# alexkroman/tiny-audio

Measured on AMD Instinct MI355X. Metric: training audio-sec/sec on 10s@16kHz clips, higher is better.
Workload: dtype bf16

## Files before the change

### include/ta355.h

```cpp
#ifndef TA355_H
#define TA355_H

#ifdef __cplusplus
extern "C" {
#endif

#ifndef __HIP_PLATFORM_AMD__
typedef struct ihipStream_t* hipStream_t;
#endif

#define TA_OK 0
#define TA_ERR_ARG 1
#define TA_ERR_LAUNCH 2

int ta_version(void);



long ta_logmel_scratch_floats(int B, int Ls, int n_mels);
int ta_logmel_mel_ranges(const float* melfb, int n_mels, int* mel_ranges, hipStream_t st);
int ta_logmel_f32(const float* wav, const long* lens, int B, int Ls, const float* dft, const float* window,
                  const float* melfb, int n_mels, float* feats, int* mask, float* scratch, const int* mel_ranges, hipStream_t st);

typedef struct {
// ... 224 lines not shown
                             const int* kmask, const int* seg, int B, int Hq, int Hkv, int L, float scale, float eps,
                             hipStream_t st);
int ta_attention_bwd_seg(const void* Q, const void* K, const void* V, const void* dO, long dO_stride, const float* LSE,
                         const float* Delta, const int* kmask, const int* seg, void* dQ, void* dK, void* dV, int B, int Hq,
                         int Hkv, int L, int Lp, float scale, hipStream_t st);
int ta_attention_bwd_qkv_seg(const void* Q, const void* K, const void* V, const void* dO, long dO_stride, const float* LSE,
                             const float* Delta, const int* kmask, const int* seg, const void* qkv0, const float* rq,
                             const float* rk, const float* qn_w, const float* kn_w, const float* cosT, const float* sinT,
                             const int* pos, void* dqkv, int B, int Hq, int Hkv, int L, int Lp, float scale, hipStream_t st);
int ta_lora_dropout_keep(const ta_lora_dropout* drop, int layer, int linear, int M, int in, unsigned char* out, hipStream_t st);


int ta_attention_enc_fwd(const void* qkv, void* out, int B, int heads, int S, hipStream_t st);

int ta_gemm_bf16_nt(const void* A, const void* W, void* C, int M, int N, int K, long lda, int a_rpb, long a_bs,
                    long ldc, int c_rpb, long c_bs, long c_off, const float* bias, const float* residual, int act,
                    int out_bf16, int splits, float* splitk_ws, hipStream_t st);
int ta_gemm_bf16_nt_ex(const void* A, const void* W, void* C, int M, int N, int K, long lda, int a_rpb, long a_bs,
                       long ldc, int c_rpb, long c_bs, long c_off, const float* bias, const float* residual, int act,
                       int out_bf16, int splits, float* splitk_ws, const int* a_idx, const int* seg,
                       const int* krange, hipStream_t st);
typedef struct {
  const void* a2; const void* w2; int k2; long lda2;
  const void* residual_bf16;
  const float* rope_tab; int rope_rows;
  int w_blocked;
  int rope_cols;
} ta_gemm_opts;
int ta_gemm_bf16_nt_opt(const void* A, const void* W, void* C, int M, int N, int K, long lda, int a_rpb, long a_bs,
                        long ldc, int c_rpb, long c_bs, long c_off, const float* bias, const float* residual, int act,
                        int out_bf16, int splits, float* splitk_ws, const int* a_idx, const int* seg,
                        const int* krange, const ta_gemm_opts* opts, hipStream_t st);
long ta_gemm_splitk_ws_bytes(int M, int N, int splits);
int ta_gemm_bf16_nt_grouped(const void* A, const void* W, void* C, int M, int N, int K, const float* bias, int act, int out_bf16,
                            const int* a_idx, const int* seg, const int* krange, int n_groups, long w_stride, long c_stride,
                            hipStream_t st);
long ta_gemm_bf16_tn_ws_bytes(int M, int Ny, int Nx);
int ta_gemm_bf16_tn(const void* Y, const void* X, float* out, int M, int Ny, int Nx, int accumulate, void* ws, long ws_bytes,
                    hipStream_t st);
int ta_profile_gemm(int enable);
int ta_profile_gemm_collect(double* total_ms, double* total_flops, long* launches);
long ta_profile_gemm_log(long* out, long max_rows);
int ta_gemm_reload_knobs(void);

int ta_layernorm_f32(const float* x, const float* w, const float* b, void* y_bf16, float* y_f32,
                     const float* rowscale, int M, int H, float eps, hipStream_t st);
int ta_layernorm_bf16(const void* x_bf16, const float* w, const float* b, void* y_bf16, float* y_f32, const float* rowscale,
                      int M, int H, float eps, hipStream_t st);
int ta_rmsnorm_fwd(const float* x, const float* w, void* y_bf16, float* y_f32, float* rstd, int M, int H,
                   float eps, int act_gelu, hipStream_t st);
int ta_rmsnorm_bwd(const float* dy, const float* x, const float* rstd, const float* w, const float* dres,
                   float* dx_f32, void* dx_bf16, float* dw_accum, int M, int H, int act_gelu, hipStream_t st);
int ta_rmsnorm_fwd_bf16(const void* x_bf16, const float* w, void* y_bf16, float* y_f32, float* rstd, int M, int H, float eps,
                        hipStream_t st);
int ta_rmsnorm_bwd_bf16(const void* dy, int dy_is_bf16, const void* x_bf16, const float* rstd, const float* w,
                        const float* dres, float* dx_f32, void* dx_bf16, int M, int H, hipStream_t st);
int ta_rmsnorm_bwd_bf16s(const void* dy, int dy_is_bf16, const void* x_bf16, const float* rstd, const float* w,
                         const void* dres_bf16, float* dx_f32, void* dx_bf16, int M, int H, hipStream_t st);
int ta_rmsnorm_bwd_dyb(const void* dy_bf16, const float* x, const float* rstd, const float* w, const float* dres, float* dx_f32,
                       void* dx_bf16, int M, int H, hipStream_t st);

int ta_rmsnorm_dw(const void* dy, int dy_is_bf16, const void* x, int x_is_bf16, const float* rstd, float* dw_accum, int M,
                  int H, hipStream_t st);

int ta_attention_fwd(const void* Q, const void* K, const void* VT, void* O, float* LSE, const int* kmask, int B,
                     int Hq, int Hkv, int L, int Lp, int head_dim, int causal, float scale, hipStream_t st);
// ... 81 lines not shown
```

### tiny_audio_amd/csrc/api.hip

```cpp
#include <cstdlib>
#include "common.h"
#include "internal.h"
#include "../../include/ta355.h"

extern "C" int ta_version(void) { return 4; }

#include <algorithm>
#include "host_util.h"


namespace {
struct EncDesc {
  int H, F, L, nh, NM, max_pos, k1;
  float eps;
  const void *conv1_w, *conv2_w;
  const float *conv1_b, *conv2_b, *norm_w, *norm_b;
  const float *rope_cos, *rope_sin, *rope_il, *pos_emb;
  const ta_enc_layer* layers;
  int res_f32;
  bool whisper;
};
EncDesc enc_desc(const ta_encoder_weights* w) {
  return EncDesc{w->hidden, w->ffn, w->n_layers, w->heads, w->n_mels, w->max_pos, 3 * w->n_mels, w->ln_eps, w->conv1_w, w->conv2_w,
                 w->conv1_b, w->conv2_b, w->norm_w, w->norm_b, w->rope_cos, w->rope_sin, w->rope_il, nullptr, w->layers, w->res_f32, false};
// ... 271 lines not shown
  s.xn = c.take<bf16_t>((size_t)d.M * d.D);
  s.act = c.take<bf16_t>((size_t)d.M * d.F);
  s.hl = c.take<bf16_t>((size_t)nl * d.D);
  s.logits = c.take<float>((size_t)nl * w->vocab_pad);
  s.dhl = c.take<float>((size_t)nl * d.D);
  s.dhn = c.take<float>((size_t)d.M * d.D);
  s.dxa = c.take<float>((size_t)d.M * d.D);
  s.dxb32 = c.take<float>((size_t)d.M * d.D);
  s.dxn = c.take<float>((size_t)d.M * d.D);
  s.dxb = c.take<bf16_t>((size_t)d.M * d.D);
  s.dact = c.take<bf16_t>((size_t)d.M * d.F);
  s.dgu = c.take<bf16_t>((size_t)d.M * 2 * d.F);
  s.dao = c.take<bf16_t>((size_t)d.M * d.nq * d.hd);
  s.dot = nullptr;
  s.delta = c.take<float>((size_t)B * d.nq * L);
  s.dq = c.take<bf16_t>((size_t)d.M * d.nq * d.hd);
  s.dk = c.take<bf16_t>((size_t)d.M * d.nkv * d.hd);
  s.dv = c.take<bf16_t>((size_t)d.M * d.nkv * d.hd);
  s.dqkv = c.take<bf16_t>((size_t)d.M * d.NQKV);
  s.dyB = c.take<bf16_t>((size_t)d.M * 64);
  s.lora_part = nullptr; s.lp_layer = 0;
  if (w->lora_rank > 0) {
    const int r = w->lora_rank, bq = d.nq * d.hd;
    const int members[4] = {3, 1, 2, 1}, Ng[4] = {d.NQKV, d.D, 2 * d.F, d.D}, ing[4] = {d.D, bq, d.D, d.F};
    long off = 0;
    for (int g = 0; g < 4; ++g) {
      const int chunks = ta_cdiv((int)d.M, ta_i_lora_tn2_rows((int)d.M, Ng[g], ing[g]));
      s.lp_size[2 * g] = (long)members[g] * r * ing[g]; s.lp_size[2 * g + 1] = (long)Ng[g] * r;
      for (int h = 0; h < 2; ++h) { s.lp_chunks[2 * g + h] = chunks; s.lp_off[2 * g + h] = off; off += s.lp_size[2 * g + h] * chunks; }
    }
    s.lp_layer = off;
    s.lora_part = c.take<float>((size_t)off * w->n_layers);
  }
  const int sp = pick_splits(nl, d.D, w->vocab_pad);
  s.skws = c.take<float>((size_t)ta_gemm_splitk_ws_bytes(nl, d.D, sp) / 4 + 4);
  s.tA = s.tB = nullptr; s.wsk = nullptr;
  if (w->train_base) {
    const int Kp = pad64((int)d.M), Kl = pad64(nl), bq = d.nq * d.hd;
    const size_t a_rows = (size_t)std::max(std::max(2 * d.F, d.NQKV), d.D), b_rows = (size_t)std::max(std::max(d.F, bq), d.D);
    s.tA = c.take<bf16_t>(std::max(a_rows * Kp, (size_t)w->vocab_pad * Kl));
    s.tB = c.take<bf16_t>(std::max(b_rows * Kp, (size_t)d.D * Kl));
    const int shp[4][2] = {{d.NQKV, d.D}, {d.D, bq}, {2 * d.F, d.D}, {d.D, d.F}};
    size_t mx = 0;
    for (auto& q : shp) {
      mx = std::max(mx, (size_t)ta_gemm_splitk_ws_bytes(q[0], q[1], wgrad_splits(q[0], q[1], Kp)));
      mx = std::max(mx, (size_t)ta_gemm_bf16_tn_ws_bytes((int)d.M, q[0], q[1]));
    }
    s.wsk = c.take<float>(mx / 4 + 4);
  }
  s.bytes = c.total();
  return s;
}
}

extern "C" long ta_lm_tape_bytes(const ta_lm_weights* w, int B, int L, int n_label_rows) {
  LmLayerTape store[MAX_LM_LAYERS];
  if (w->n_layers > MAX_LM_LAYERS) return -1;
  return (long)lm_tape(w, B, L, n_label_rows, nullptr, store).bytes;
}
extern "C" long ta_lm_workspace_bytes(const ta_lm_weights* w, int B, int L, int n_label_rows) {
  return (long)lm_ws(w, B, L, n_label_rows, nullptr).bytes;
}

static int lm_layers_forward(const ta_lm_weights* w, const LmDims& d, int B, int L, const int* kmask, const int* pos,
                             LmLayerTape* store, bool alias, float* x_final, LmWs& s, const ta_i_lora_layer_imgs* ext,
                             bf16_t* kcache, bf16_t* vcache, int Lmax, hipStream_t st, const LoraDropDev* drop = nullptr,
                             const int* seg = nullptr) {
// ... 296 lines not shown
  }
  if (n_lab <= 0) {
    if (d_embeds && hipMemsetAsync(d_embeds, 0, (size_t)M * d.D * 4, st) != hipSuccess) return TA_ERR_LAUNCH;
    return TA_OK;
  }
  ta_gemm_opts kx = opts_none();
  LoraDrop pend{};
  const bf16_t* pend_at = nullptr;
  auto lora_bwd = [&](const bf16_t* dy, int N, const bf16_t* x, int in, const bf16_t* xa, const LoraImg& g, float* dla,
                      float* dlb, int members, int b0, int b1, int layer, int grp) -> int {
    static const int lj_base[4] = {0, 3, 4, 6};
    RC(ta_i_lora_skinny_nt(dy, N, g.bt, s.dyB, M, members * r, st));
    float* pb = lora_parts ? s.lora_part + (long)layer * s.lp_layer + s.lp_off[2 * grp + 1] : nullptr;
    float* pa = lora_parts ? s.lora_part + (long)layer * s.lp_layer + s.lp_off[2 * grp] : nullptr;
    if (dp) {
      pend = LoraDrop{*dp, (unsigned)(8 * layer + lj_base[grp]), r, members};
      RC(ta_i_lora_skinny_tn2(dy, N, xa, members * r, dlb, r, 1, 1.0f, r, b0, b1, x, in, s.dyB, members * r, dla, 1, in,
                              w->lora_scale * dp->inv_keep, 0, 0, 0, M, pb, s.lp_size[2 * grp + 1], pa, s.lp_size[2 * grp], st, &pend));
      pend_at = g.at;
      return TA_OK;
    }
    RC(ta_i_lora_skinny_tn2(dy, N, xa, members * r, dlb, r, 1, 1.0f, r, b0, b1, x, in, s.dyB, members * r, dla, 1, in, w->lora_scale,
                            0, 0, 0, M, pb, s.lp_size[2 * grp + 1], pa, s.lp_size[2 * grp], st));
    kx = opts_kext(s.dyB, g.at);
    return TA_OK;
  };
  auto take_ext = [&]() { const ta_gemm_opts o = kx; kx = opts_none(); return o; };
  auto dx_drop_term = [&](void* out, int in) -> int {
    if (!pend_at) return TA_OK;
    const bf16_t* at = pend_at;
    pend_at = nullptr;
    return ta_i_lora_dx_drop(s.dyB, at, out, M, in, pend, st);
  };
  const int sp = pick_splits(n_lab, d.D, w->vocab_pad);
  RC(ta_gemm_bf16_nt(t.dlogits, w->embed_t_bf16, s.dhl, n_lab, d.D, w->vocab_pad, w->vocab_pad, 0, 0, d.D, 0, 0, 0, nullptr,
                     nullptr, 0, 0, sp, s.skws, st));
  if (hipMemsetAsync(s.dhn, 0, (size_t)M * d.D * 4, st) != hipSuccess) return TA_ERR_LAUNCH;
  RC(ta_scatter_rows_f32(s.dhl, label_rows, s.dhn, n_lab, d.D, st));
  const int Kp = pad64(M);
  auto wgrad = [&](const bf16_t* dy, int n_out, const bf16_t* x, int k_in, float* dW) -> int {
    if (!dW) return TA_OK;
    if (n_out <= 4096 && k_in <= 2048)
      return ta_gemm_bf16_tn(dy, x, dW, M, n_out, k_in, 1, s.wsk, ta_gemm_bf16_tn_ws_bytes(M, n_out, k_in), st);
    RC(ta_transpose_to_bf16(dy, 0, n_out, 0, 0, s.tA, Kp, M, n_out, st));
    RC(ta_transpose_to_bf16(x, 0, k_in, 0, 0, s.tB, Kp, M, k_in, st));
    return ta_gemm_bf16_nt(s.tA, s.tB, dW, n_out, k_in, Kp, Kp, 0, 0, k_in, 0, 0, 0, nullptr, dW, 0, 0,
                           wgrad_splits(n_out, k_in, Kp), s.wsk, st);
  };
  if (wg) {
    if (wg->dembed) {
      const int Kl = pad64(n_lab);
      RC(ta_gather_rows_bf16(t.hn, label_rows, s.hl, n_lab, d.D, st));
      RC(ta_transpose_to_bf16(t.dlogits, 0, w->vocab_pad, 0, 0, s.tA, Kl, n_lab, w->vocab_pad, st));
      RC(ta_transpose_to_bf16(s.hl, 0, d.D, 0, 0, s.tB, Kl, n_lab, d.D, st));
      RC(ta_gemm_bf16_nt(s.tA, s.tB, wg->dembed, w->vocab, d.D, Kl, Kl, 0, 0, d.D, 0, 0, 0, nullptr, wg->dembed, 0, 0, 1,
                         nullptr, st));
    }
    if (wg->dnorm) RC(ta_rmsnorm_dw(s.dhn, 0, t.x_final, lm_res_bf16(w), t.r_f, wg->dnorm, M, d.D, st));
  }
  float* dx = s.dxa;
  float* dx_alt = s.dxb32;
  const int gb = 1;
  const bool dx_bf16 = lm_res_bf16(w) && w->dx_f32 == 0;
  auto norm_bwd = [&](const float* dy, int dyb, const float* x, const float* r, const float* gw, const float* dres, float* dxf,
                      bool last = false) -> int {
    if (dx_bf16) return ta_rmsnorm_bwd_bf16s(dy, dyb, x, r, gw, dres ? s.dxb : nullptr, last ? dxf : nullptr, s.dxb, M, d.D, st);
    if (lm_res_bf16(w)) return ta_rmsnorm_bwd_bf16(dy, dyb, x, r, gw, dres, dxf, s.dxb, M, d.D, st);
// ... 68 lines not shown
```

### tiny_audio_amd/csrc/common.h

```cpp
#pragma once
#include <hip/hip_runtime.h>
#include <stdint.h>

typedef uint16_t bf16_t;
typedef __attribute__((ext_vector_type(8))) short bf16x8;
typedef __attribute__((ext_vector_type(4))) short bf16x4;
typedef __attribute__((ext_vector_type(4))) float f32x4;

#define TA_OK 0
#define TA_ERR_ARG 1
#define TA_ERR_LAUNCH 2

#define TA_LAUNCH(...)                \
  do {                                \
    (void)hipGetLastError();          \
    hipLaunchKernelGGL(__VA_ARGS__);  \
  } while (0)

#define TA_CHECK_LAUNCH()                                  \
  do {                                                     \
    hipError_t e__ = hipGetLastError();                    \
    if (e__ != hipSuccess) return TA_ERR_LAUNCH;           \
  } while (0)

__device__ __forceinline__ float bf2f(bf16_t v) { return __uint_as_float(((uint32_t)v) << 16); }

typedef __attribute__((ext_vector_type(2))) __bf16 ta_bf2_t;
typedef __attribute__((ext_vector_type(2))) float ta_f2_t;
__device__ __forceinline__ uint32_t pack2bf(float lo, float hi) {
  ta_f2_t v = {lo, hi};
  ta_bf2_t b = __builtin_convertvector(v, ta_bf2_t);
  return __builtin_bit_cast(uint32_t, b);
}
__device__ __forceinline__ bf16_t f2bf(float f) { return (bf16_t)(pack2bf(f, 0.f) & 0xffffu); }

__device__ __forceinline__ float wave_sum(float v) {
#pragma unroll
  for (int o = 32; o > 0; o >>= 1) v += __shfl_xor(v, o, 64);
  return v;
}
__device__ __forceinline__ float wave_max(float v) {
#pragma unroll
  for (int o = 32; o > 0; o >>= 1) v = fmaxf(v, __shfl_xor(v, o, 64));
  return v;
}

__device__ __forceinline__ float gelu_erf(float x) { return 0.5f * x * (1.0f + erff(x * 0.70710678118654752f)); }
__device__ __forceinline__ float gelu_erf_grad(float x) {
  return 0.5f * (1.0f + erff(x * 0.70710678118654752f)) + x * 0.3989422804014327f * __expf(-0.5f * x * x);
}

__device__ __forceinline__ float gelu_erf_fast(float x) {
  const float z = x * 0.70710678118654752f, az = fabsf(z);
  const float t = __builtin_amdgcn_rcpf(fmaf(0.3275911f, az, 1.0f));
  float p = fmaf(1.061405429f, t, -1.453152027f);
  p = fmaf(p, t, 1.421413741f);
  p = fmaf(p, t, -0.284496736f);
  p = fmaf(p, t, 0.254829592f);
  const float e = __builtin_amdgcn_exp2f(-az * az * 1.4426950408889634f);
  const float erfz = copysignf(1.0f - p * t * e, z);
  return 0.5f * x * (1.0f + erfz);
}

static inline int ta_cdiv(long a, long b) { return (int)((a + b - 1) / b); }
```

### tiny_audio_amd/csrc/elementwise.hip

```cpp
#include "common.h"

static inline int ew_blocks(long n, int per_block = 256) {
  long b = (n + per_block - 1) / per_block;
  return (int)(b > 4096 ? 4096 : (b < 1 ? 1 : b));
}

__global__ void swiglu_fwd_kernel(const bf16_t* __restrict__ gu, bf16_t* __restrict__ act, long M, int F) {
  const long n4 = M * (F / 4);
  for (long i = (long)blockIdx.x * blockDim.x + threadIdx.x; i < n4; i += (long)gridDim.x * blockDim.x) {
    const long m = i / (F / 4); const int c = (int)(i % (F / 4)) * 4;
    const uint2 gv = *(const uint2*)(gu + m * 2 * F + c);
    const uint2 uv = *(const uint2*)(gu + m * 2 * F + F + c);
    const float g[4] = {bf2f(gv.x & 0xffff), bf2f(gv.x >> 16), bf2f(gv.y & 0xffff), bf2f(gv.y >> 16)};
    const float u[4] = {bf2f(uv.x & 0xffff), bf2f(uv.x >> 16), bf2f(uv.y & 0xffff), bf2f(uv.y >> 16)};
    float a[4];
#pragma unroll
    for (int j = 0; j < 4; ++j) a[j] = g[j] / (1.f + __expf(-g[j])) * u[j];
    uint2 o; o.x = pack2bf(a[0], a[1]); o.y = pack2bf(a[2], a[3]);
    *(uint2*)(act + m * F + c) = o;
  }
}
__global__ void swiglu_bwd_kernel(const bf16_t* __restrict__ dact, const bf16_t* __restrict__ gu,
                                  bf16_t* __restrict__ dgu, long M, int F) {
  const long n4 = M * (F / 4);
// ... 112 lines not shown

template <bool F32>
__global__ __launch_bounds__(256) void pos_add_kernel(void* __restrict__ xv, const float* __restrict__ pos, long n_chunks, long per_clip) {
  for (long i = (long)blockIdx.x * blockDim.x + threadIdx.x; i < n_chunks; i += (long)gridDim.x * blockDim.x) {
    const long j = i % per_clip;
    if constexpr (F32) {
      float4 v = ((const float4*)xv)[i];
      const float4 p = ((const float4*)pos)[j];
      v.x += p.x; v.y += p.y; v.z += p.z; v.w += p.w;
      ((float4*)xv)[i] = v;
    } else {
      const uint4 v = ((const uint4*)xv)[i];
      const float4 p0 = ((const float4*)pos)[2 * j], p1 = ((const float4*)pos)[2 * j + 1];
      uint4 o;
      o.x = pack2bf(bf2f(v.x & 0xffff) + p0.x, bf2f(v.x >> 16) + p0.y);
      o.y = pack2bf(bf2f(v.y & 0xffff) + p0.z, bf2f(v.y >> 16) + p0.w);
      o.z = pack2bf(bf2f(v.z & 0xffff) + p1.x, bf2f(v.z >> 16) + p1.y);
      o.w = pack2bf(bf2f(v.w & 0xffff) + p1.z, bf2f(v.w >> 16) + p1.w);
      ((uint4*)xv)[i] = o;
    }
  }
}
extern "C" int ta_pos_add(void* x, int x_f32, const float* pos, int B, int S, int H, hipStream_t st) {
  if (B <= 0 || S <= 0) return TA_OK;
  if (!x || !pos || H <= 0 || (H % 8)) return TA_ERR_ARG;
  const long per_clip = (long)S * H / (x_f32 ? 4 : 8), n = per_clip * B;
  if (x_f32) TA_LAUNCH((pos_add_kernel<true>), dim3(ew_blocks(n)), dim3(256), 0, st, x, pos, n, per_clip);
  else TA_LAUNCH((pos_add_kernel<false>), dim3(ew_blocks(n)), dim3(256), 0, st, x, pos, n, per_clip);
  TA_CHECK_LAUNCH(); return TA_OK;
}

__global__ __launch_bounds__(1024) void audio_index_kernel(const long* __restrict__ ids, const long* __restrict__ counts,
                                                           int* __restrict__ src_row, int B, int L, int N, long audio_id) {
  __shared__ int scan[1024];
  __shared__ int carry;
  __shared__ long cum[1025];
  const int tid = threadIdx.x;
  if (tid == 0) {
    carry = 0; cum[0] = 0;
    for (int i = 0; i < B && i < 1024; ++i) cum[i + 1] = cum[i] + counts[i];
  }
  __syncthreads();
  const int total = B * L;
  for (int base = 0; base < total; base += 1024) {
    const int p = base + tid;
    const int flag = (p < total && ids[p] == audio_id) ? 1 : 0;
    scan[tid] = flag;
    __syncthreads();
    for (int o = 1; o < 1024; o <<= 1) {
      const int v = tid >= o ? scan[tid - o] : 0;
      __syncthreads();
      scan[tid] += v;
      __syncthreads();
    }
    if (p < total) {
      int out = -1;
      if (flag) {
        const long rank = carry + scan[tid] - 1;
        int lo = 0, hi = B;
        while (hi - lo > 1) { const int mid = (lo + hi) >> 1; if (cum[mid] <= rank) lo = mid; else hi = mid; }
        const long n = rank - cum[lo];
        out = (rank < cum[B] && n < N) ? (int)(lo * N + n) : -2;
      }
      src_row[p] = out;
    }
    __syncthreads();
    if (tid == 1023) carry += scan[1023];
    __syncthreads();
  }
}
__global__ __launch_bounds__(256) void segment_table_kernel(const int* __restrict__ sid, int* __restrict__ seg_start,
                                                            int* __restrict__ seg_end, int* __restrict__ pos, int R, int L) {
  const long p = (long)blockIdx.x * 256 + threadIdx.x;
  if (p >= (long)R * L) return;
  const int l = (int)(p % L);
  const int* row = sid + (p - l);
  const int s = row[l];
  int a = l, e = l + 1;
  if (s == 0) { a = l + 1; e = l; }
  else {
    while (a > 0 && row[a - 1] == s) --a;
    while (e < L && row[e] == s) ++e;
  }
  seg_start[p] = a;
  seg_end[p] = e;
  if (pos) pos[p] = s == 0 ? 0 : l - a;
}
__global__ __launch_bounds__(256) void audio_index_seg_kernel(const long* __restrict__ ids, const int* __restrict__ sid,
                                                              const long* __restrict__ counts, int* __restrict__ src_row, int R, int L,
                                                              int C_, int N, long audio_id) {
  __shared__ int clip0;
  const int r = blockIdx.x;
  if (threadIdx.x == 0) {
    int c = 0;
    for (int i = 0; i < r; ++i) { int m = 0; for (int l = 0; l < L; ++l) m = max(m, sid[(long)i * L + l]); c += m; }
    clip0 = c;
  }
  __syncthreads();
  const int* srow = sid + (long)r * L;
  const long* irow = ids + (long)r * L;
  for (int l = threadIdx.x; l < L; l += 256) {
// ... 218 lines not shown
```

### tiny_audio_amd/csrc/gemm.hip

```cpp
#include "gemm_common.h"

template <int ACT, bool OUT_BF16, bool HAS_RES, int BMT = 128, bool KEXT = false>
__global__ __launch_bounds__(256, 2) void gemm_nt_kernel(GemmArgs p) {
  constexpr int MI = BMT / 32, WR = BMT / 2;
  __shared__ __attribute__((aligned(16))) char smem[4 * TILE_BYTES];
  const int tid = threadIdx.x, lane = tid & 63, wave = tid >> 6;
  const int wm = wave >> 1, wn = wave & 1;
  const int g = lane >> 4, l15 = lane & 15;

  const int nwg = gridDim.x;
  int bid = blockIdx.x;
  {
    const int q = nwg >> 3, r = nwg & 7, xcd = bid & 7, within = bid >> 3;
    bid = (xcd < r ? xcd * (q + 1) : r * (q + 1) + (xcd - r) * q) + within;
  }
  const int tiles = p.tiles_m * p.tiles_n;
  const int z = bid / tiles;
  int t = bid - z * tiles;
  const int GROUP_M = p.group_m > 0 ? p.group_m : 8;
  const int width = GROUP_M * p.tiles_n;
  const int group = t / width;
  const int first_m = group * GROUP_M;
  const int gsize = min(p.tiles_m - first_m, GROUP_M);
  int pm = first_m + (t % width) % gsize;
// ... 642 lines not shown
  const bool wide = epilogue_wide_ok(p);
  const float2* lut = stage_gelu_lut<ACT, 256>(smem, p, tid, true);
  if (res_init) epilogue_tile<6, 4, ACT, OUT_BF16, false>(acc, p, Cb, m0 + wm * 96 + l15, Mact, rbase, n0 + wn * 64, g, wide, biasp, lut);
  else epilogue_tile<6, 4, ACT, OUT_BF16, HAS_RES, ((HAS_RES && !OUT_BF16) ? 3 : 2)>(acc, p, Cb, m0 + wm * 96 + l15, Mact, rbase, n0 + wn * 64, g, wide, biasp, lut);
}

#include <vector>
namespace {
struct ProfRec { hipEvent_t a, b; double flops; };
bool g_prof_on = false;
std::vector<ProfRec> g_prof;
#define TA_GEMM_LOG_FIELDS 24
bool g_log_on = false;
std::vector<long> g_log;
}

#include <cstdlib>
struct GemmKnobs {
  int variant;
  int gelu_erf;
  void load() {
    auto i = [](const char* n, int d) { const char* v = getenv(n); return (v && *v) ? atoi(v) : d; };
    variant = i("TA355_GEMM_VARIANT", -1);
    gelu_erf = i("TA355_GELU_LUT", 1) == 0;
  }
};
static GemmKnobs& knobs() {
  static GemmKnobs k = [] { GemmKnobs x; x.load(); return x; }();
  return k;
}
void ta_i_reload_decode_knobs();
extern "C" int ta_gemm_reload_knobs(void) { knobs().load(); ta_i_reload_decode_knobs(); return TA_OK; }

static int pick_variant(int M, int N, int K, int splits) {
  const int forced = knobs().variant;
  if (forced >= 0 && forced <= 12 && !(forced >= 6 && forced <= 9) && forced != 11) return forced;
  const double rate[6] = {1.0, TA355_RATE_256x256, TA355_RATE_256x128, TA355_RATE_256x256_PP, TA355_RATE_256x320_PP, TA355_RATE_96x128};
  const int bm[6] = {128, 256, 256, 256, 256, 96}, bn[6] = {128, 256, 128, 256, 320, 128}, slots[6] = {512, 256, 256, 256, 256, 512};
  int best = 0; double best_t = 1e300;
  for (int v = 0; v < 6; ++v) {
    const long tiles = (long)ta_cdiv(M, bm[v]) * ta_cdiv(N, bn[v]) * splits;
    const double rounds = (double)((tiles + slots[v] - 1) / slots[v]);
    const double t = rounds * (double)bm[v] * bn[v] / rate[v] * ((v == 0 || v == 5) ? 2.0 : 1.0);
    if (t < best_t) { best_t = t; best = v; }
  }
  {
    const long tiles = (long)ta_cdiv(M, 192) * ta_cdiv(N, 128) * splits;
    const double t = (double)((tiles + 255) / 256) * 192.0 * 128.0 / TA355_RATE_192x128;
    if (TA355_RATE_192x128 > 0.0 && K / splits >= 2048 && t < best_t) { best_t = t; best = 10; }
  }
  {
    const long tiles = (long)ta_cdiv(M, 192) * ta_cdiv(N, 256) * splits;
    const double t = (double)((tiles + 255) / 256) * 192.0 * 256.0 / TA355_RATE_192x256_PP;
    if (TA355_RATE_192x256_PP > 0.0 && K / splits >= 128 && t < best_t) { best_t = t; best = 12; }
  }
  return best;
}

template <int ACT, bool OUT_BF16, bool HAS_RES, bool KEXT>
static void launch_variant(int variant, bool persist, int grid, int pgrid, const GemmArgs& a, hipStream_t st) {
  if (variant == 0) TA_LAUNCH((gemm_nt_kernel<ACT, OUT_BF16, HAS_RES, 128, KEXT>), dim3(grid), dim3(256), 0, st, a);
  else if (variant == 5) TA_LAUNCH((gemm_nt_kernel<ACT, OUT_BF16, HAS_RES, 96, KEXT>), dim3(grid), dim3(256), 0, st, a);
  else if (variant == 1) TA_LAUNCH((gemm_nt_kernel_v2<256, ACT, OUT_BF16, HAS_RES, false, KEXT>), dim3(grid), dim3(512), 0, st, a);
  else if (variant == 12) TA_LAUNCH((gemm_nt_kernel_v4<256, ACT, OUT_BF16, HAS_RES, 192>), dim3(pgrid), dim3(512), 0, st, a);
  else if (variant == 3 && persist) TA_LAUNCH((gemm_nt_kernel_v4<256, ACT, OUT_BF16, HAS_RES>), dim3(pgrid), dim3(512), 0, st, a);
  else if (variant == 4 && persist) TA_LAUNCH((gemm_nt_kernel_v4<320, ACT, OUT_BF16, HAS_RES>), dim3(pgrid), dim3(512), 0, st, a);
  else if (variant == 3) TA_LAUNCH((gemm_nt_kernel_v2<256, ACT, OUT_BF16, HAS_RES, true, KEXT>), dim3(grid), dim3(512), 0, st, a);
  else if (variant == 4) TA_LAUNCH((gemm_nt_kernel_v2<320, ACT, OUT_BF16, HAS_RES, true, KEXT>), dim3(grid), dim3(512), 0, st, a);
  else if (variant == 10) TA_LAUNCH((gemm_nt_kernel_v5<ACT, OUT_BF16, HAS_RES, KEXT>), dim3(grid), dim3(256), 0, st, a);
  else TA_LAUNCH((gemm_nt_kernel_v2<128, ACT, OUT_BF16, HAS_RES, false, KEXT>), dim3(grid), dim3(512), 0, st, a);
}

template <int ACT, bool OUT_BF16, bool HAS_RES>
static int launch_gemm(GemmArgs a, hipStream_t st) {
  if (a.A2 && ACT != 0) return TA_ERR_ARG;
  int variant = pick_variant(a.M, a.N, a.K, a.splits);
  const bool a_far = !a.a_plain && ((long)(a.M / a.a_rpb + 1) * a.a_bs + a.lda * a.a_rpb) * 2 >= (1L << 32);
  if (variant == 10 && (a.w_blocked || a.a_idx || a_far)) variant = 5;
  if (variant == 12 && (a.a_idx || a_far || a.A2)) variant = 3;
  const int bm = variant == 0 ? 128 : (variant == 5 ? 96 : ((variant == 10 || variant == 12) ? 192 : 256));
  const int bn = variant == 4 ? 320 : ((variant == 1 || variant == 3 || variant == 12) ? 256 : 128);
  a.tiles_m = ta_cdiv(a.M, bm) + ((a.grp_n > 0 && a.seg) ? a.grp_n : 0); a.tiles_n = ta_cdiv(a.N, bn);
  const int grid = a.tiles_m * a.tiles_n * a.splits;
  a.group_m = (variant != 0 && a.tiles_m <= 8) ? a.tiles_m : 0;
  a.wide = (((long)a.N | a.ldc | a.c_off | a.c_bs) & 7) == 0;
  a.gelu_erf = knobs().gelu_erf;
  const bool persist = (variant == 3 || variant == 4) && !a.a_idx && !a.A2 && !a_far;
  static const int ncu = [] { int dev = 0, n = 0; (void)hipGetDevice(&dev); (void)hipDeviceGetAttribute(&n, hipDeviceAttributeMultiprocessorCount, dev); return n > 0 ? n : 256; }();
  const int pgrid = grid < ncu ? grid : ncu;
// ... 168 lines not shown
```

### tiny_audio_amd/csrc/host_util.h

```cpp
#pragma once
#include "common.h"
#include "internal.h"
#include "../../include/ta355.h"

namespace {
struct Carver {
  char* base; size_t off;
  explicit Carver(void* b) : base((char*)b), off(0) {}
  template <typename T> T* take(size_t n) {
    off = (off + 255) & ~(size_t)255;
    T* p = base ? (T*)(base + off) : nullptr;
    off += n * sizeof(T);
    return p;
  }
  size_t total() const { return (off + 255) & ~(size_t)255; }
};
inline int pad64(int x) { return (x + 63) / 64 * 64; }
inline int gemm(const void* A, const void* W, void* C, int M, int N, int K, const float* bias, const float* res, int act,
                int out_bf16, hipStream_t st) {
  return ta_gemm_bf16_nt(A, W, C, M, N, K, K, 0, 0, N, 0, 0, 0, bias, res, act, out_bf16, 1, nullptr, st);
}
inline int gemm_opt(const void* A, const void* W, void* C, int M, int N, int K, const float* bias, const float* res, int act,
                    int out_bf16, const ta_gemm_opts& o, hipStream_t st) {
  return ta_gemm_bf16_nt_opt(A, W, C, M, N, K, K, 0, 0, N, 0, 0, 0, bias, res, act, out_bf16, 1, nullptr, nullptr, nullptr, nullptr,
                             &o, st);
}
inline ta_gemm_opts opts_none() { return ta_gemm_opts{nullptr, nullptr, 0, 0, nullptr, nullptr, 0, 0, 0}; }
inline ta_gemm_opts opts_kext(const void* a2, const void* w2) { ta_gemm_opts o = opts_none(); o.a2 = a2; o.w2 = w2; o.k2 = 64; o.lda2 = 64; return o; }
inline int pick_splits(int M, int N, int K) {
  const long tiles = (long)ta_cdiv(M, 128) * ta_cdiv(N, 128);
  int s = 1;
  while (tiles * s < 512 && K / 64 / (s * 2) >= 8 && s < 64) s *= 2;
  return s;
}
#define RC(x) do { int rc__ = (x); if (rc__) return rc__; } while (0)
inline size_t lora_imgs_carve(const ta_lm_weights* w, void* base, ta_i_lora_layer_imgs* out) {
  Carver c(base);
  const int D = w->hidden, F = w->ffn, bq = w->heads * w->head_dim, NQKV = (w->heads + 2 * w->kv_heads) * w->head_dim;
  const int in[4] = {D, bq, D, F}, N[4] = {NQKV, D, 2 * F, D};
  for (int l = 0; l < w->n_layers; ++l)
    for (int g = 0; g < 4; ++g) {
      LoraImg im;
      im.a = c.take<bf16_t>((size_t)64 * in[g]); im.at = c.take<bf16_t>((size_t)64 * in[g]);
      im.b = c.take<bf16_t>((size_t)64 * N[g]); im.bt = c.take<bf16_t>((size_t)64 * N[g]);
      if (out) out[l].g[g] = im;
    }
  return c.total();
}
}
```

### tiny_audio_amd/csrc/loss.hip

```cpp
#include "common.h"

template <typename T> __device__ __forceinline__ float4 ld4(const T* p);
template <> __device__ __forceinline__ float4 ld4<float>(const float* p) { return *(const float4*)p; }
template <> __device__ __forceinline__ float4 ld4<bf16_t>(const bf16_t* p) {
  const uint2 v = *(const uint2*)p;
  return make_float4(bf2f(v.x & 0xffff), bf2f(v.x >> 16), bf2f(v.y & 0xffff), bf2f(v.y >> 16));
}

template <typename T>
__global__ __launch_bounds__(256) void ce_fwd_bwd_kernel(const T* __restrict__ logits, long ldl, const int* __restrict__ rows,
                                                         const long* __restrict__ targets, int V, float scale,
                                                         float* __restrict__ nll_out, float* __restrict__ loss_accum,
                                                         bf16_t* __restrict__ dlogits, long ldd) {
  __shared__ float red_m[4], red_s[4];
  const int i = blockIdx.x, tid = threadIdx.x, lane = tid & 63, wave = tid >> 6;
  const long tgt = targets[i];
  const T* row = logits + (long)(rows ? rows[i] : i) * ldl;
  const int nv = V / 4;
  float m = -INFINITY, s = 0.f;
  for (int c = tid; c < nv; c += 256) {
    const float4 v = ld4<T>(row + c * 4);
    const float mx = fmaxf(fmaxf(v.x, v.y), fmaxf(v.z, v.w));
    if (mx > m) { s *= __expf(m - mx); m = mx; }
    s += __expf(v.x - m) + __expf(v.y - m) + __expf(v.z - m) + __expf(v.w - m);
  }
  for (int c = nv * 4 + tid; c < V; c += 256) {
    const float v = sizeof(T) == 4 ? (float)((const float*)row)[c] : bf2f(((const bf16_t*)row)[c]);
    if (v > m) { s *= __expf(m - v); m = v; }
    s += __expf(v - m);
  }
#pragma unroll
  for (int o = 32; o > 0; o >>= 1) {
    const float m2 = __shfl_xor(m, o, 64), s2 = __shfl_xor(s, o, 64);
    const float mn = fmaxf(m, m2);
    s = (m == -INFINITY ? 0.f : s * __expf(m - mn)) + (m2 == -INFINITY ? 0.f : s2 * __expf(m2 - mn));
    m = mn;
  }
  if (lane == 0) { red_m[wave] = m; red_s[wave] = s; }
  __syncthreads();
  float M = fmaxf(fmaxf(red_m[0], red_m[1]), fmaxf(red_m[2], red_m[3]));
  float S = 0.f;
#pragma unroll
  for (int w = 0; w < 4; ++w) S += red_m[w] == -INFINITY ? 0.f : red_s[w] * __expf(red_m[w] - M);
  const float lse = M + __logf(S);
  const bool valid = tgt >= 0 && tgt < V;
  if (tid == 0) {
    float nll = 0.f;
    if (valid) {
      const float zt = sizeof(T) == 4 ? (float)((const float*)row)[tgt] : bf2f(((const bf16_t*)row)[tgt]);
      nll = lse - zt;
      if (loss_accum) atomicAdd(loss_accum, nll * scale);
    }
    if (nll_out) nll_out[i] = nll;
  }
  if (!dlogits) return;
  bf16_t* drow = dlogits + (long)i * ldd;
  const float sc = valid ? scale : 0.f;
  const int nvd = (int)(ldd / 4);
  for (int c = tid; c < nvd; c += 256) {
    float o[4] = {0.f, 0.f, 0.f, 0.f};
    if (c * 4 + 3 < V) {
      const float4 v = ld4<T>(row + c * 4);
      o[0] = __expf(v.x - lse) * sc; o[1] = __expf(v.y - lse) * sc; o[2] = __expf(v.z - lse) * sc; o[3] = __expf(v.w - lse) * sc;
    } else {
      for (int j = 0; j < 4; ++j) {
        const int cc = c * 4 + j;
        if (cc < V) {
          const float v = sizeof(T) == 4 ? (float)((const float*)row)[cc] : bf2f(((const bf16_t*)row)[cc]);
          o[j] = __expf(v - lse) * sc;
        }
      }
    }
    if (valid && (long)c * 4 <= tgt && tgt < (long)c * 4 + 4) o[tgt - (long)c * 4] -= sc;
    uint2 w; w.x = pack2bf(o[0], o[1]); w.y = pack2bf(o[2], o[3]);
    *(uint2*)(drow + c * 4) = w;
  }
}

__global__ __launch_bounds__(1024) void label_rows_kernel(const long* __restrict__ labels, int B, int L,
                                                          int* __restrict__ rows, long* __restrict__ targets,
                                                          int* __restrict__ n_out) {
  __shared__ int scan[1024];
  __shared__ int carry;
  const int tid = threadIdx.x;
  if (tid == 0) carry = 0;
  __syncthreads();
  const int total = B * L;
  for (int base = 0; base < total; base += 1024) {
    const int p = base + tid;
    long t = -100;
    if (p < total) { const int l = p % L; if (l + 1 < L) t = labels[p + 1]; }
    const int flag = (t != -100) ? 1 : 0;
    scan[tid] = flag;
    __syncthreads();
    for (int o = 1; o < 1024; o <<= 1) {
      const int v = tid >= o ? scan[tid - o] : 0;
      __syncthreads();
      scan[tid] += v;
      __syncthreads();
    }
    if (flag) { const int k = carry + scan[tid] - 1; rows[k] = p; targets[k] = t; }
    __syncthreads();
    if (tid == 1023) carry += scan[1023];
    __syncthreads();
  }
  if (tid == 0) n_out[0] = carry;
}

__global__ __launch_bounds__(1024) void nll_sum_kernel(const float* __restrict__ nll, int n, float scale, float* __restrict__ loss_accum) {
  __shared__ float red[16];
  float s = 0.f;
  for (int i = threadIdx.x; i < n; i += 1024) s += nll[i] * scale;
  s = wave_sum(s);
  if ((threadIdx.x & 63) == 0) red[threadIdx.x >> 6] = s;
  __syncthreads();
  if (threadIdx.x == 0) {
    float t = 0.f;
    for (int w = 0; w < 16; ++w) t += red[w];
    loss_accum[0] += t;
  }
}

extern "C" int ta_cross_entropy(const void* logits, int logits_bf16, long ldl, const int* rows, const long* targets,
                                int n, int V, float scale, float* nll, float* loss_accum, void* dlogits_bf16, long ldd,
                                hipStream_t st) {
  if (n <= 0) return TA_OK;
  if ((ldl % 4) || (dlogits_bf16 && (ldd % 4))) return TA_ERR_ARG;
  float* atomic_loss = nll ? nullptr : loss_accum;
  if (logits_bf16)
    TA_LAUNCH((ce_fwd_bwd_kernel<bf16_t>), dim3(n), dim3(256), 0, st, (const bf16_t*)logits, ldl, rows, targets, V,
                       scale, nll, atomic_loss, (bf16_t*)dlogits_bf16, ldd);
  else
    TA_LAUNCH((ce_fwd_bwd_kernel<float>), dim3(n), dim3(256), 0, st, (const float*)logits, ldl, rows, targets, V,
                       scale, nll, atomic_loss, (bf16_t*)dlogits_bf16, ldd);
  TA_CHECK_LAUNCH();
  if (loss_accum && nll) {
    TA_LAUNCH(nll_sum_kernel, dim3(1), dim3(1024), 0, st, nll, n, scale, loss_accum);
    TA_CHECK_LAUNCH();
  }
// ... 10 lines not shown
```

Measured before the change: 7599.

## Add cost-model split-K planner, wave-level block scans, and unrolled CE loops

Adds a split-K planner that scores candidate split counts with the variant cost model plus a reduction penalty, and uses it for the LM-head dgrad GEMM. Replaces the serial 1024-wide shared-memory Hillis-Steele scans in label_rows and audio_index with a two-level wavefront shuffle scan, each thread handling a contiguous chunk. Unrolls the cross-entropy forward and backward loops 8-way so several loads are in flight at once, and simplifies the target check. The scan changes cut sync-heavy small kernels; the split-K change may alter GEMM time and the size of the workspace it needs.

```diff
diff --git a/include/ta355.h b/include/ta355.h
--- a/include/ta355.h
+++ b/include/ta355.h
@@ -280,6 +280,7 @@
                         int out_bf16, int splits, float* splitk_ws, const int* a_idx, const int* seg,
                         const int* krange, const ta_gemm_opts* opts, hipStream_t st);
 long ta_gemm_splitk_ws_bytes(int M, int N, int splits);
+int ta_gemm_plan(int M, int N, int K, int splits_default, int* variant, int* splits);
 int ta_gemm_bf16_nt_grouped(const void* A, const void* W, void* C, int M, int N, int K, const float* bias, int act, int out_bf16,
                             const int* a_idx, const int* seg, const int* krange, int n_groups, long w_stride, long c_stride,
                             hipStream_t st);
diff --git a/tiny_audio_amd/csrc/api.hip b/tiny_audio_amd/csrc/api.hip
--- a/tiny_audio_amd/csrc/api.hip
+++ b/tiny_audio_amd/csrc/api.hip
@@ -327,7 +327,7 @@
     s.lp_layer = off;
     s.lora_part = c.take<float>((size_t)off * w->n_layers);
   }
-  const int sp = pick_splits(nl, d.D, w->vocab_pad);
+  const int sp = pick_splits_plain(nl, d.D, w->vocab_pad);
   s.skws = c.take<float>((size_t)ta_gemm_splitk_ws_bytes(nl, d.D, sp) / 4 + 4);
   s.tA = s.tB = nullptr; s.wsk = nullptr;
   if (w->train_base) {
@@ -690,7 +690,7 @@
     pend_at = nullptr;
     return ta_i_lora_dx_drop(s.dyB, at, out, M, in, pend, st);
   };
-  const int sp = pick_splits(n_lab, d.D, w->vocab_pad);
+  const int sp = pick_splits_plain(n_lab, d.D, w->vocab_pad);
   RC(ta_gemm_bf16_nt(t.dlogits, w->embed_t_bf16, s.dhl, n_lab, d.D, w->vocab_pad, w->vocab_pad, 0, 0, d.D, 0, 0, 0, nullptr,
                      nullptr, 0, 0, sp, s.skws, st));
   if (hipMemsetAsync(s.dhn, 0, (size_t)M * d.D * 4, st) != hipSuccess) return TA_ERR_LAUNCH;
diff --git a/tiny_audio_amd/csrc/common.h b/tiny_audio_amd/csrc/common.h
--- a/tiny_audio_amd/csrc/common.h
+++ b/tiny_audio_amd/csrc/common.h
@@ -45,6 +45,27 @@
   return v;
 }
 
+template <typename T>
+__device__ __forceinline__ T block_scan_excl_1024(T v, T* sm, T* total) {
+  const int tid = threadIdx.x, lane = tid & 63, wave = tid >> 6;
+  T inc = v;
+#pragma unroll
+  for (int o = 1; o < 64; o <<= 1) { const T t = __shfl_up(inc, o, 64); if (lane >= o) inc += t; }
+  if (lane == 63) sm[wave] = inc;
+  __syncthreads();
+  if (wave == 0) {
+    const T w = lane < 16 ? sm[lane] : (T)0;
+    T wi = w;
+#pragma unroll
+    for (int o = 1; o < 16; o <<= 1) { const T t = __shfl_up(wi, o, 64); if (lane >= o) wi += t; }
+    if (lane < 16) sm[lane] = wi - w;
+    if (lane == 15) sm[16] = wi;
+  }
+  __syncthreads();
+  *total = sm[16];
+  return sm[wave] + inc - v;
+}
+
 __device__ __forceinline__ float gelu_erf(float x) { return 0.5f * x * (1.0f + erff(x * 0.70710678118654752f)); }
 __device__ __forceinline__ float gelu_erf_grad(float x) {
   return 0.5f * (1.0f + erff(x * 0.70710678118654752f)) + x * 0.3989422804014327f * __expf(-0.5f * x * x);
diff --git a/tiny_audio_amd/csrc/elementwise.hip b/tiny_audio_amd/csrc/elementwise.hip
--- a/tiny_audio_amd/csrc/elementwise.hip
+++ b/tiny_audio_amd/csrc/elementwise.hip
@@ -168,41 +168,31 @@
 
 __global__ __launch_bounds__(1024) void audio_index_kernel(const long* __restrict__ ids, const long* __restrict__ counts,
                                                            int* __restrict__ src_row, int B, int L, int N, long audio_id) {
-  __shared__ int scan[1024];
-  __shared__ int carry;
-  __shared__ long cum[1025];
+  __shared__ int sm_i[17];
+  __shared__ long long sm_l[17];
+  __shared__ long long cum[1025];
   const int tid = threadIdx.x;
-  if (tid == 0) {
-    carry = 0; cum[0] = 0;
-    for (int i = 0; i < B && i < 1024; ++i) cum[i + 1] = cum[i] + counts[i];
-  }
-  __syncthreads();
-  const int total = B * L;
-  for (int base = 0; base < total; base += 1024) {
-    const int p = base + tid;
-    const int flag = (p < total && ids[p] == audio_id) ? 1 : 0;
-    scan[tid] = flag;
-    __syncthreads();
-    for (int o = 1; o < 1024; o <<= 1) {
-      const int v = tid >= o ? scan[tid - o] : 0;
-      __syncthreads();
-      scan[tid] += v;
-      __syncthreads();
-    }
-    if (p < total) {
-      int out = -1;
-      if (flag) {
-        const long rank = carry + scan[tid] - 1;
-        int lo = 0, hi = B;
-        while (hi - lo > 1) { const int mid = (lo + hi) >> 1; if (cum[mid] <= rank) lo = mid; else hi = mid; }
-        const long n = rank - cum[lo];
-        out = (rank < cum[B] && n < N) ? (int)(lo * N + n) : -2;
-      }
-      src_row[p] = out;
-    }
-    __syncthreads();
-    if (tid == 1023) carry += scan[1023];
-    __syncthreads();
+  const long long cnt = tid < B ? (long long)counts[tid] : 0;
+  long long cum_all;
+  const long long cex = block_scan_excl_1024<long long>(cnt, sm_l, &cum_all);
+  if (tid < B) cum[tid] = cex;
+  if (tid == 0) cum[B] = cum_all;
+  const int total = B * L, per = (total + 1023) / 1024;
+  const int p0 = min(tid * per, total), p1 = min(p0 + per, total);
+  int mine = 0;
+  for (int p = p0; p < p1; ++p) mine += ids[p] == audio_id;
+  int all;
+  long long rank = block_scan_excl_1024<int>(mine, sm_i, &all);
+  for (int p = p0; p < p1; ++p) {
+    int out = -1;
+    if (ids[p] == audio_id) {
+      int lo = 0, hi = B;
+      while (hi - lo > 1) { const int mid = (lo + hi) >> 1; if (cum[mid] <= rank) lo = mid; else hi = mid; }
+      const long long n = rank - cum[lo];
+      out = (rank < cum[B] && n < N) ? (int)(lo * N + n) : -2;
+      ++rank;
+    }
+    src_row[p] = out;
   }
 }
 __global__ __launch_bounds__(256) void segment_table_kernel(const int* __restrict__ sid, int* __restrict__ seg_start,
diff --git a/tiny_audio_amd/csrc/gemm.hip b/tiny_audio_amd/csrc/gemm.hip
--- a/tiny_audio_amd/csrc/gemm.hip
+++ b/tiny_audio_amd/csrc/gemm.hip
@@ -698,7 +698,7 @@
 void ta_i_reload_decode_knobs();
 extern "C" int ta_gemm_reload_knobs(void) { knobs().load(); ta_i_reload_decode_knobs(); return TA_OK; }
 
-static int pick_variant(int M, int N, int K, int splits) {
+static int pick_variant(int M, int N, int K, int splits, double* cost_out = nullptr) {
   const int forced = knobs().variant;
   if (forced >= 0 && forced <= 12 && !(forced >= 6 && forced <= 9) && forced != 11) return forced;
   const double rate[6] = {1.0, TA355_RATE_256x256, TA355_RATE_256x128, TA355_RATE_256x256_PP, TA355_RATE_256x320_PP, TA355_RATE_96x128};
@@ -720,7 +720,27 @@
     const double t = (double)((tiles + 255) / 256) * 192.0 * 256.0 / TA355_RATE_192x256_PP;
     if (TA355_RATE_192x256_PP > 0.0 && K / splits >= 128 && t < best_t) { best_t = t; best = 12; }
   }
+  if (cost_out) *cost_out = best_t;
   return best;
+}
+
+#define TA355_FILL_MIN_K 4096
+extern "C" int ta_gemm_plan(int M, int N, int K, int splits_default, int* variant, int* splits) {
+  if (M <= 0 || N <= 0 || K <= 0 || (K % BK) || !splits) return TA_ERR_ARG;
+  int best_s = splits_default > 1 ? splits_default : 1, best_v = -1;
+  if (K >= TA355_FILL_MIN_K && knobs().variant < 0) {
+    double best_t = 1e300;
+    const int s_hi = std::min(64, K / TA355_FILL_MIN_K);
+    for (int s = 1; s <= s_hi; ++s) {
+      double area = 0.0;
+      const int v = pick_variant(M, N, K, s, &area);
+      const double t = area * (double)(K / BK) / s + (s > 1 ? (double)s * M * N / 16.0 : 0.0);
+      if (t < best_t) { best_t = t; best_s = s; best_v = v; }
+    }
+  }
+  if (variant) *variant = best_v;
+  *splits = best_s;
+  return TA_OK;
 }
 
 template <int ACT, bool OUT_BF16, bool HAS_RES, bool KEXT>
diff --git a/tiny_audio_amd/csrc/host_util.h b/tiny_audio_amd/csrc/host_util.h
--- a/tiny_audio_amd/csrc/host_util.h
+++ b/tiny_audio_amd/csrc/host_util.h
@@ -33,6 +33,11 @@
   while (tiles * s < 512 && K / 64 / (s * 2) >= 8 && s < 64) s *= 2;
   return s;
 }
+inline int pick_splits_plain(int M, int N, int K) {
+  int s = 1;
+  if (ta_gemm_plan(M, N, K, pick_splits(M, N, K), nullptr, &s) != TA_OK) return pick_splits(M, N, K);
+  return s;
+}
 #define RC(x) do { int rc__ = (x); if (rc__) return rc__; } while (0)
 inline size_t lora_imgs_carve(const ta_lm_weights* w, void* base, ta_i_lora_layer_imgs* out) {
   Carver c(base);
diff --git a/tiny_audio_amd/csrc/loss.hip b/tiny_audio_amd/csrc/loss.hip
--- a/tiny_audio_amd/csrc/loss.hip
+++ b/tiny_audio_amd/csrc/loss.hip
@@ -18,12 +18,21 @@
   const T* row = logits + (long)(rows ? rows[i] : i) * ldl;
   const int nv = V / 4;
   float m = -INFINITY, s = 0.f;
-  for (int c = tid; c < nv; c += 256) {
-    const float4 v = ld4<T>(row + c * 4);
+  auto fold = [&](const float4 v) {
     const float mx = fmaxf(fmaxf(v.x, v.y), fmaxf(v.z, v.w));
     if (mx > m) { s *= __expf(m - mx); m = mx; }
     s += __expf(v.x - m) + __expf(v.y - m) + __expf(v.z - m) + __expf(v.w - m);
+  };
+  constexpr int CE_U = 8;
+  int c = tid;
+  for (; c + (CE_U - 1) * 256 < nv; c += CE_U * 256) {
+    float4 v[CE_U];
+#pragma unroll
+    for (int u = 0; u < CE_U; ++u) v[u] = ld4<T>(row + (c + u * 256) * 4);
+#pragma unroll
+    for (int u = 0; u < CE_U; ++u) fold(v[u]);
   }
+  for (; c < nv; c += 256) fold(ld4<T>(row + c * 4));
   for (int c = nv * 4 + tid; c < V; c += 256) {
     const float v = sizeof(T) == 4 ? (float)((const float*)row)[c] : bf2f(((const bf16_t*)row)[c]);
     if (v > m) { s *= __expf(m - v); m = v; }
@@ -57,21 +66,36 @@
   bf16_t* drow = dlogits + (long)i * ldd;
   const float sc = valid ? scale : 0.f;
   const int nvd = (int)(ldd / 4);
-  for (int c = tid; c < nvd; c += 256) {
+  const int ct = valid ? (int)(tgt >> 2) : -1, jt = (int)(tgt & 3);
+  auto emit = [&](int cc, const float4 v) {
+    float o[4] = {__expf(v.x - lse) * sc, __expf(v.y - lse) * sc, __expf(v.z - lse) * sc, __expf(v.w - lse) * sc};
+    if (cc == ct) {
+#pragma unroll
+      for (int j = 0; j < 4; ++j) if (j == jt) o[j] -= sc;
+    }
+    uint2 w; w.x = pack2bf(o[0], o[1]); w.y = pack2bf(o[2], o[3]);
+    *(uint2*)(drow + cc * 4) = w;
+  };
+  const int nfull = nv < nvd ? nv : nvd;
+  c = tid;
+  for (; c + (CE_U - 1) * 256 < nfull; c += CE_U * 256) {
+    float4 v[CE_U];
+#pragma unroll
+    for (int u = 0; u < CE_U; ++u) v[u] = ld4<T>(row + (c + u * 256) * 4);
+#pragma unroll
+    for (int u = 0; u < CE_U; ++u) emit(c + u * 256, v[u]);
+  }
+  for (; c < nfull; c += 256) emit(c, ld4<T>(row + c * 4));
+  for (c = nfull + tid; c < nvd; c += 256) {
     float o[4] = {0.f, 0.f, 0.f, 0.f};
-    if (c * 4 + 3 < V) {
-      const float4 v = ld4<T>(row + c * 4);
-      o[0] = __expf(v.x - lse) * sc; o[1] = __expf(v.y - lse) * sc; o[2] = __expf(v.z - lse) * sc; o[3] = __expf(v.w - lse) * sc;
-    } else {
-      for (int j = 0; j < 4; ++j) {
-        const int cc = c * 4 + j;
-        if (cc < V) {
-          const float v = sizeof(T) == 4 ? (float)((const float*)row)[cc] : bf2f(((const bf16_t*)row)[cc]);
-          o[j] = __expf(v - lse) * sc;
-        }
+    for (int j = 0; j < 4; ++j) {
+      const int cc = c * 4 + j;
+      if (cc < V) {
+        const float v = sizeof(T) == 4 ? (float)((const float*)row)[cc] : bf2f(((const bf16_t*)row)[cc]);
+        o[j] = __expf(v - lse) * sc;
       }
     }
-    if (valid && (long)c * 4 <= tgt && tgt < (long)c * 4 + 4) o[tgt - (long)c * 4] -= sc;
+    if (c == ct) o[jt] -= sc;
     uint2 w; w.x = pack2bf(o[0], o[1]); w.y = pack2bf(o[2], o[3]);
     *(uint2*)(drow + c * 4) = w;
   }
@@ -80,31 +104,20 @@
 __global__ __launch_bounds__(1024) void label_rows_kernel(const long* __restrict__ labels, int B, int L,
                                                           int* __restrict__ rows, long* __restrict__ targets,
                                                           int* __restrict__ n_out) {
-  __shared__ int scan[1024];
-  __shared__ int carry;
+  __shared__ int sm[17];
   const int tid = threadIdx.x;
-  if (tid == 0) carry = 0;
-  __syncthreads();
-  const int total = B * L;
-  for (int base = 0; base < total; base += 1024) {
-    const int p = base + tid;
-    long t = -100;
-    if (p < total) { const int l = p % L; if (l + 1 < L) t = labels[p + 1]; }
-    const int flag = (t != -100) ? 1 : 0;
-    scan[tid] = flag;
-    __syncthreads();
-    for (int o = 1; o < 1024; o <<= 1) {
-      const int v = tid >= o ? scan[tid - o] : 0;
-      __syncthreads();
-      scan[tid] += v;
-      __syncthreads();
-    }
-    if (flag) { const int k = carry + scan[tid] - 1; rows[k] = p; targets[k] = t; }
-    __syncthreads();
-    if (tid == 1023) carry += scan[1023];
-    __syncthreads();
+  const int total = B * L, per = (total + 1023) / 1024;
+  const int p0 = min(tid * per, total), p1 = min(p0 + per, total);
+  auto target = [&](int p) -> long { return (p % L) + 1 < L ? labels[p + 1] : -100; };
+  int mine = 0;
+  for (int p = p0; p < p1; ++p) mine += target(p) != -100;
+  int all;
+  int k = block_scan_excl_1024<int>(mine, sm, &all);
+  for (int p = p0; p < p1; ++p) {
+    const long t = target(p);
+    if (t != -100) { rows[k] = p; targets[k] = t; ++k; }
   }
-  if (tid == 0) n_out[0] = carry;
+  if (tid == 0) n_out[0] = all;
 }
 
 __global__ __launch_bounds__(1024) void nll_sum_kernel(const float* __restrict__ nll, int n, float scale, float* __restrict__ loss_accum) {
```

Measured after the change: 7625 (median of 6 runs). About the same (+0.3%).
